# AlmondGod/diffusion-piano

Hardware: AMD Instinct MI355X
Metric: env steps/sec at 4096 parallel envs; qpos L∞ drift vs CPU MuJoCo (higher is better)
Workload: dtype f32; 1 GPU; 4096 envs/GPU crossing_field random-action rollout, 10 physics substeps per env-step, constraint forces by the primal Newton solve (friction loss, uncapped rows); envs_per_gpu=4096, song=crossing_field, parallelism=dp1

## Files before the change

### diffusion-piano_amd/csrc/collide_x.h

```cpp
#pragma once
#include "prims.h"

namespace ps {

struct XShape {
  int type;
  f3 c;
  float R[9];
  f3 p0, p1;
  float r;
  f3 hs;
  int v0, nv;
  f3 e0, e1;
  float er;
  const uint64_t* cells;
  const float4* cellv;
  float tie;
};

constexpr float SUP_TIE_HULL = 2e-6f;
constexpr float SUP_TIE_BOX = 1e-6f;
constexpr float SUP_TIE_CAP = 1e-6f;

__device__ __forceinline__ void x_shift(XShape& s, f3 o) {
  s.c = s.c - o;
  s.p0 = s.p0 - o;
  s.p1 = s.p1 - o;
  s.e0 = s.e0 - o;
  s.e1 = s.e1 - o;
}

__device__ __forceinline__ void quat_to_R(float w, float x, float y, float z, float* R) {
  const float n = rsqrtf(w * w + x * x + y * y + z * z);
  w *= n; x *= n; y *= n; z *= n;
  R[0] = 1.f - 2.f * (y * y + z * z); R[1] = 2.f * (x * y - w * z); R[2] = 2.f * (x * z + w * y);
  R[3] = 2.f * (x * y + w * z); R[4] = 1.f - 2.f * (x * x + z * z); R[5] = 2.f * (y * z - w * x);
  R[6] = 2.f * (x * z - w * y); R[7] = 2.f * (y * z + w * x); R[8] = 1.f - 2.f * (x * x + y * y);
}
__device__ __forceinline__ void R_to_quat(const float* R, float* q) {
  const float t = R[0] + R[4] + R[8];
  if (t > 0.f) {
    const float s = sqrtf(t + 1.f) * 2.f, i = 1.f / s;
    q[0] = 0.25f * s; q[1] = (R[7] - R[5]) * i; q[2] = (R[2] - R[6]) * i; q[3] = (R[3] - R[1]) * i;
  } else if (R[0] > R[4] && R[0] > R[8]) {
    const float s = sqrtf(1.f + R[0] - R[4] - R[8]) * 2.f, i = 1.f / s;
    q[0] = (R[7] - R[5]) * i; q[1] = 0.25f * s; q[2] = (R[1] + R[3]) * i; q[3] = (R[2] + R[6]) * i;
  } else if (R[4] > R[8]) {
    const float s = sqrtf(1.f + R[4] - R[0] - R[8]) * 2.f, i = 1.f / s;
    q[0] = (R[2] - R[6]) * i; q[1] = (R[1] + R[3]) * i; q[2] = 0.25f * s; q[3] = (R[5] + R[7]) * i;
  } else {
    const float s = sqrtf(1.f + R[8] - R[0] - R[4]) * 2.f, i = 1.f / s;
    q[0] = (R[3] - R[1]) * i; q[1] = (R[2] + R[6]) * i; q[2] = (R[5] + R[7]) * i; q[3] = 0.25f * s;
  }
}

__device__ __forceinline__ float sgn0f(float x) { return x > 0.f ? 1.f : (x < 0.f ? -1.f : 0.f); }
__device__ __forceinline__ f3 nrmz3(f3 a) {
  const float n = norm3(a);
  return n > 0.f ? a * (1.f / n) : a;
}

__device__ __forceinline__ int hull_cell(f3 d) {
  const float ex = fabsf(d.x), ey = fabsf(d.y), ez = fabsf(d.z);
  int ax;
  float mj, a, b;
  if (ex >= ey && ex >= ez) { ax = 0; mj = d.x; a = d.y; b = d.z; }
  else if (ey >= ez) { ax = 1; mj = d.y; a = d.z; b = d.x; }
  else { ax = 2; mj = d.z; a = d.x; b = d.y; }
  const float inv = 1.f / fabsf(mj), hg = 0.5f * XCG;
  const int ia = (int)fminf(fmaxf(fmaf(a, inv, 1.f) * hg, 0.f), XCG - 1.f);
  const int ib = (int)fminf(fmaxf(fmaf(b, inv, 1.f) * hg, 0.f), XCG - 1.f);
  return ((2 * ax + (mj < 0.f ? 1 : 0)) * XCG + ia) * XCG + ib;
}

__device__ __forceinline__ float sgn_tie(float x, float band) { return fabsf(x) <= band ? 0.f : sgn0f(x); }
__device__ __forceinline__ f3 x_support_local(const DevModel* __restrict__ m, const XShape& s, f3 d) {
  const f3 dl = mtv3(s.R, d);
  f3 loc;
  if (s.type == PS_GEOM_BOX) {
    const float band = SUP_TIE_BOX * fmaxf(fabsf(dl.x), fmaxf(fabsf(dl.y), fabsf(dl.z)));
    loc = mk3(sgn_tie(dl.x, band) * s.hs.x, sgn_tie(dl.y, band) * s.hs.y, sgn_tie(dl.z, band) * s.hs.z);
  } else if (s.cellv) {
    const bool zero = dl.x == 0.f && dl.y == 0.f && dl.z == 0.f;
    const float4* t = s.cellv + (zero ? XNCELL : hull_cell(dl)) * XCV;
    float4 v[XCV];
#pragma unroll
    for (int u = 0; u < XCV; u++) v[u] = t[u];
    const float tie = s.tie * norm3(dl);
    float bd = -INFINITY;
    loc = mk3(0.f, 0.f, 0.f);
#pragma unroll
    for (int u = 0; u < XCV; u++) {
      const float p = fmaf(dl.z, v[u].z, fmaf(dl.y, v[u].y, dl.x * v[u].x));
      if (p > bd + tie) { bd = p; loc = mk3(v[u].x, v[u].y, v[u].z); }
    }
  } else if (s.cells) {
    const bool zero = dl.x == 0.f && dl.y == 0.f && dl.z == 0.f;
    uint64_t msk = zero ? 1ull : s.cells[hull_cell(dl)];
    const float tie = s.tie * norm3(dl);
    float bd = -INFINITY;
    loc = mk3(0.f, 0.f, 0.f);
    while (msk) {
      bool ok[4];
      f3 v[4];
#pragma unroll
      for (int u = 0; u < 4; u++) {
        ok[u] = msk != 0ull;
        const int id = ok[u] ? __builtin_ctzll(msk) : 0;
        msk &= msk - 1ull;
        const float4 q = *reinterpret_cast<const float4*>(m->hull_v[s.v0 + id]);
        v[u] = mk3(q.x, q.y, q.z);
      }
#pragma unroll
      for (int u = 0; u < 4; u++) {
        const float p = fmaf(dl.z, v[u].z, fmaf(dl.y, v[u].y, dl.x * v[u].x));
        if (ok[u] && p > bd + tie) { bd = p; loc = v[u]; }
      }
    }
  } else {
    const float tie = s.tie * norm3(dl);
    float bd = -INFINITY;
    loc = mk3(0.f, 0.f, 0.f);
    for (int i0 = 0; i0 < s.nv; i0 += 8) {
      float4 v[8];
#pragma unroll
      for (int j = 0; j < 8; j++) v[j] = *reinterpret_cast<const float4*>(m->hull_v[s.v0 + min(i0 + j, s.nv - 1)]);
#pragma unroll
      for (int j = 0; j < 8; j++) {
        const float p = fmaf(dl.z, v[j].z, fmaf(dl.y, v[j].y, dl.x * v[j].x));
        if (i0 + j < s.nv && p > bd + tie) { bd = p; loc = mk3(v[j].x, v[j].y, v[j].z); }
      }
    }
  }
  return loc;
}
__device__ __forceinline__ f3 x_support(const DevModel* __restrict__ m, const XShape& s, f3 d) {
  if (s.type == 0) {
    const f3 ax = s.p1 - s.p0;
    const float dn = norm3(d);
    float da = dot3(ax, d);
    if (fabsf(da) <= SUP_TIE_CAP * norm3(ax) * dn) da = 0.f;
    const f3 base = da > 0.f ? s.p1 : (da < 0.f ? s.p0 : (s.p0 + s.p1) * 0.5f);
    return dn > 0.f ? base + d * (s.r / dn) : base;
  }
  return s.c + mv3(s.R, x_support_local(m, s, d));
}

constexpr float MPR_TOLF = 1e-6f;
constexpr int MPR_MAXITF = 50;
constexpr float MPR_EPSF = 2.220446049250313e-16f;
struct MprPt {
  f3 v, a, b;
};
__device__ __forceinline__ bool mpr_zero(float x) { return fabsf(x) < MPR_EPSF; }
__device__ __forceinline__ MprPt mpr_sup(const DevModel* __restrict__ m, const XShape& A, const XShape& B, f3 d) {
  MprPt p;
  p.a = x_support(m, A, d);
  p.b = x_support(m, B, d * -1.f);
  p.v = p.a - p.b;
  return p;
}
__device__ __forceinline__ float xchg1(float v) {
  return __int_as_float(__builtin_amdgcn_update_dpp(0, __float_as_int(v), 0xB1, 0xF, 0xF, false));
}
template <bool PAIR>
__device__ __forceinline__ MprPt mpr_sup_t(const DevModel* __restrict__ m, const XShape& A, const XShape& B,
                                           const XShape& O, bool role, f3 d) {
  if (!PAIR) return mpr_sup(m, A, B, d);
  const f3 mine = x_support(m, O, role ? d * -1.f : d);
  const f3 oth = mk3(xchg1(mine.x), xchg1(mine.y), xchg1(mine.z));
  MprPt p;
  p.a = role ? oth : mine;
  p.b = role ? mine : oth;
  p.v = p.a - p.b;
  return p;
}
__device__ __forceinline__ f3 portal_dir(const MprPt& p1, const MprPt& p2, const MprPt& p3) {
  return nrmz3(cross3(p2.v - p1.v, p3.v - p1.v));
}
__device__ __forceinline__ bool portal_reach_tol(const MprPt& p1, const MprPt& p2, const MprPt& p3, const MprPt& v4, f3 dir) {
  const float d4 = dot3(v4.v, dir);
  const float mn = fminf(d4 - dot3(p1.v, dir), fminf(d4 - dot3(p2.v, dir), d4 - dot3(p3.v, dir)));
  return mn <= MPR_TOLF;
}
__device__ __forceinline__ void expand_portal(const MprPt& p0, MprPt& p1, MprPt& p2, MprPt& p3, const MprPt& v4) {
  const f3 v4v0 = cross3(v4.v, p0.v);
  if (dot3(p1.v, v4v0) > 0.f) {
    if (dot3(p2.v, v4v0) > 0.f) p1 = v4; else p3 = v4;
  } else {
    if (dot3(p3.v, v4v0) > 0.f) p2 = v4; else p1 = v4;
  }
}
__device__ __forceinline__ f3 tri_closest_origin_d(f3 af, f3 bf, f3 cf) {
  const double ax = af.x, ay = af.y, az = af.z, bx = bf.x, by = bf.y, bz = bf.z, cx = cf.x, cy = cf.y, cz = cf.z;
  const double abx = bx - ax, aby = by - ay, abz = bz - az, acx = cx - ax, acy = cy - ay, acz = cz - az;
  const double d1 = -(abx * ax + aby * ay + abz * az), d2 = -(acx * ax + acy * ay + acz * az);
  if (d1 <= 0.0 && d2 <= 0.0) return af;
  const double d3 = -(abx * bx + aby * by + abz * bz), d4 = -(acx * bx + acy * by + acz * bz);
  if (d3 >= 0.0 && d4 <= d3) return bf;
  const double vc = d1 * d4 - d3 * d2;
  if (vc <= 0.0 && d1 >= 0.0 && d3 <= 0.0) {
    const double t = d1 / (d1 - d3);
    return mk3((float)(ax + abx * t), (float)(ay + aby * t), (float)(az + abz * t));
  }
  const double d5 = -(abx * cx + aby * cy + abz * cz), d6 = -(acx * cx + acy * cy + acz * cz);
  if (d6 >= 0.0 && d5 <= d6) return cf;
  const double vb = d5 * d2 - d1 * d6;
  if (vb <= 0.0 && d2 >= 0.0 && d6 <= 0.0) {
    const double t = d2 / (d2 - d6);
    return mk3((float)(ax + acx * t), (float)(ay + acy * t), (float)(az + acz * t));
  }
  const double va = d3 * d6 - d5 * d4;
  if (va <= 0.0 && (d4 - d3) >= 0.0 && (d5 - d6) >= 0.0) {
    const double t = (d4 - d3) / ((d4 - d3) + (d5 - d6));
    return mk3((float)(bx + (cx - bx) * t), (float)(by + (cy - by) * t), (float)(bz + (cz - bz) * t));
  }
  const double den = 1.0 / (va + vb + vc), v = vb * den, w = vc * den;
  return mk3((float)(ax + abx * v + acx * w), (float)(ay + aby * v + acy * w), (float)(az + abz * v + acz * w));
}
__device__ __forceinline__ f3 mpr_pos(const MprPt& p0, const MprPt& p1, const MprPt& p2, const MprPt& p3) {
  const f3 dir = portal_dir(p1, p2, p3);
  float b0 = dot3(cross3(p1.v, p2.v), p3.v), b1 = dot3(cross3(p3.v, p2.v), p0.v);
  float b2 = dot3(cross3(p0.v, p1.v), p3.v), b3 = dot3(cross3(p2.v, p1.v), p0.v);
  float sum = b0 + b1 + b2 + b3;
// ... 4 lines not shown
    b3 = dot3(cross3(p1.v, p2.v), dir);
    sum = b1 + b2 + b3;
  }
  const float inv = 1.f / sum;
  const f3 pa = p0.a * b0 + p1.a * b1 + p2.a * b2 + p3.a * b3;
  const f3 pb = p0.b * b0 + p1.b * b1 + p2.b * b2 + p3.b * b3;
  return (pa * inv + pb * inv) * 0.5f;
}
template <bool PAIR = false>
__device__ __forceinline__ int mpr_penetration(const DevModel* __restrict__ m, const XShape& A, const XShape& B,
                                               float* depth, f3* n, f3* pos, int* its = nullptr,
                                               const XShape* O = nullptr, bool role = false) {
  const XShape& own = PAIR ? *O : A;
  MprPt p0, p1, p2, p3;
  p0.a = A.c; p0.b = B.c; p0.v = A.c - B.c;
  if (p0.v.x == 0.f && p0.v.y == 0.f && p0.v.z == 0.f) p0.v.x += 10.f * MPR_EPSF;
  f3 dir = nrmz3(p0.v * -1.f);
  p1 = mpr_sup_t<PAIR>(m, A, B, own, role, dir);
  float dt = dot3(p1.v, dir);
  if (mpr_zero(dt) || dt < 0.f) return 0;
  dir = cross3(p0.v, p1.v);
  if (mpr_zero(dot3(dir, dir))) {
    *pos = (p1.a + p1.b) * 0.5f;
    if (p1.v.x == 0.f && p1.v.y == 0.f && p1.v.z == 0.f) { *depth = 0.f; *n = mk3(0.f, 0.f, 0.f); }
    else { *depth = norm3(p1.v); *n = nrmz3(p1.v); }
    return 1;
  }
  dir = nrmz3(dir);
  p2 = mpr_sup_t<PAIR>(m, A, B, own, role, dir);
  dt = dot3(p2.v, dir);
  if (mpr_zero(dt) || dt < 0.f) return 0;
  dir = nrmz3(cross3(p1.v - p0.v, p2.v - p0.v));
  if (dot3(dir, p0.v) > 0.f) { const MprPt t = p1; p1 = p2; p2 = t; dir = dir * -1.f; }
  for (int it = 0;; it++) {
    if (its) ++*its;
    if (it > 4 * MPR_MAXITF) return 0;
    p3 = mpr_sup_t<PAIR>(m, A, B, own, role, dir);
    dt = dot3(p3.v, dir);
    if (mpr_zero(dt) || dt < 0.f) return 0;
    bool cont = false;
    float t = dot3(cross3(p1.v, p3.v), p0.v);
    if (t < 0.f && !mpr_zero(t)) { p2 = p3; cont = true; }
    if (!cont) {
      t = dot3(cross3(p3.v, p2.v), p0.v);
      if (t < 0.f && !mpr_zero(t)) { p1 = p3; cont = true; }
    }
    if (!cont) break;
    dir = nrmz3(cross3(p1.v - p0.v, p2.v - p0.v));
  }
  for (int it = 0;; it++) {
    if (its) ++*its;
    if (it > 4 * MPR_MAXITF) return 0;
    dir = portal_dir(p1, p2, p3);
    dt = dot3(p1.v, dir);
    if (mpr_zero(dt) || dt > 0.f) break;
    const MprPt v4 = mpr_sup_t<PAIR>(m, A, B, own, role, dir);
    const float d4 = dot3(v4.v, dir);
    if (!(mpr_zero(d4) || d4 > 0.f) || portal_reach_tol(p1, p2, p3, v4, dir)) return 0;
    expand_portal(p0, p1, p2, p3, v4);
  }
  for (int it = 0;; it++) {
    if (its) ++*its;
    dir = portal_dir(p1, p2, p3);
    const MprPt v4 = mpr_sup_t<PAIR>(m, A, B, own, role, dir);
    if (portal_reach_tol(p1, p2, p3, v4, dir) || it > MPR_MAXITF) {
      const f3 cp = tri_closest_origin_d(p1.v, p2.v, p3.v);
      *depth = norm3(cp);
      *n = mpr_zero(*depth) ? dir : cp * (1.f / *depth);
      *pos = mpr_pos(p0, p1, p2, p3);
      return 1;
    }
    expand_portal(p0, p1, p2, p3, v4);
  }
}

struct d3 {
  double x, y, z;
};
__device__ __forceinline__ d3 mkd3(double a, double b, double c) { return {a, b, c}; }
__device__ __forceinline__ d3 tod3(f3 a) { return {a.x, a.y, a.z}; }
__device__ __forceinline__ f3 tof3(d3 a) { return mk3((float)a.x, (float)a.y, (float)a.z); }
__device__ __forceinline__ d3 operator+(d3 a, d3 b) { return {a.x + b.x, a.y + b.y, a.z + b.z}; }
__device__ __forceinline__ d3 operator-(d3 a, d3 b) { return {a.x - b.x, a.y - b.y, a.z - b.z}; }
__device__ __forceinline__ d3 operator*(d3 a, double s) { return {a.x * s, a.y * s, a.z * s}; }
__device__ __forceinline__ double dotd(d3 a, d3 b) { return a.x * b.x + a.y * b.y + a.z * b.z; }
__device__ __forceinline__ d3 crossd(d3 a, d3 b) {
  return {a.y * b.z - a.z * b.y, a.z * b.x - a.x * b.z, a.x * b.y - a.y * b.x};
}
#ifndef PS_MPR_FASTN
#define PS_MPR_FASTN 1
#endif
__device__ __forceinline__ double rsqrtd(double x) {
  const double r = (double)__frsqrt_rn((float)x);
  return r * (1.5 - 0.5 * x * r * r);
}
__device__ __forceinline__ d3 nrmzd(d3 a) {
  const double n2 = dotd(a, a);
  if (PS_MPR_FASTN && n2 > 1e-30 && n2 < 1e30) return a * rsqrtd(n2);
  const double n = sqrt(n2);
  return n > 0.0 ? a * (1.0 / n) : a;
}
__device__ __forceinline__ bool mpr_zerod(double x) { return fabs(x) < 2.220446049250313e-16; }
__device__ __forceinline__ d3 x_support_d(const DevModel* __restrict__ m, const XShape& s, d3 d) {
  if (s.type == 0) {
    const d3 p0 = tod3(s.p0), p1 = tod3(s.p1), ax = p1 - p0;
    const double dd = dotd(d, d);
// ... 16 lines not shown
struct MprPtD {
  d3 v, a, b;
};
__device__ __forceinline__ double xchg1d(double v) {
  const long long u = __double_as_longlong(v);
  const int lo = __builtin_amdgcn_update_dpp(0, (int)(u & 0xffffffffll), 0xB1, 0xF, 0xF, false);
  const int hi = __builtin_amdgcn_update_dpp(0, (int)(u >> 32), 0xB1, 0xF, 0xF, false);
  return __longlong_as_double(((long long)hi << 32) | (unsigned int)lo);
}
template <bool PAIR>
__device__ __forceinline__ MprPtD mpr_sup_d(const DevModel* __restrict__ m, const XShape& A, const XShape& B,
                                            const XShape& O, bool role, d3 d) {
  MprPtD p;
  if (!PAIR) {
    p.a = x_support_d(m, A, d);
    p.b = x_support_d(m, B, d * -1.0);
  } else {
    const d3 mine = x_support_d(m, O, role ? d * -1.0 : d);
    const d3 oth = mkd3(xchg1d(mine.x), xchg1d(mine.y), xchg1d(mine.z));
    p.a = role ? oth : mine;
    p.b = role ? mine : oth;
  }
  p.v = p.a - p.b;
  return p;
}
__device__ __forceinline__ d3 portal_dir_d(const MprPtD& p1, const MprPtD& p2, const MprPtD& p3) {
  return nrmzd(crossd(p2.v - p1.v, p3.v - p1.v));
}
__device__ __forceinline__ bool portal_reach_tol_d(const MprPtD& p1, const MprPtD& p2, const MprPtD& p3,
                                                   const MprPtD& v4, d3 dir) {
  const double d4 = dotd(v4.v, dir);
  return fmin(d4 - dotd(p1.v, dir), fmin(d4 - dotd(p2.v, dir), d4 - dotd(p3.v, dir))) <= 1e-6;
}
__device__ __forceinline__ void expand_portal_d(const MprPtD& p0, MprPtD& p1, MprPtD& p2, MprPtD& p3, const MprPtD& v4) {
  const d3 v4v0 = crossd(v4.v, p0.v);
  if (dotd(p1.v, v4v0) > 0.0) {
    if (dotd(p2.v, v4v0) > 0.0) p1 = v4; else p3 = v4;
  } else {
    if (dotd(p3.v, v4v0) > 0.0) p2 = v4; else p1 = v4;
  }
}
__device__ __forceinline__ d3 tri_closest_origin_dd(d3 a, d3 b, d3 c) {
  const d3 ab = b - a, ac = c - a;
  const double d1 = -dotd(ab, a), d2 = -dotd(ac, a);
  if (d1 <= 0.0 && d2 <= 0.0) return a;
  const double d3_ = -dotd(ab, b), d4 = -dotd(ac, b);
  if (d3_ >= 0.0 && d4 <= d3_) return b;
  const double vc = d1 * d4 - d3_ * d2;
  if (vc <= 0.0 && d1 >= 0.0 && d3_ <= 0.0) return a + ab * (d1 / (d1 - d3_));
  const double d5 = -dotd(ab, c), d6 = -dotd(ac, c);
  if (d6 >= 0.0 && d5 <= d6) return c;
  const double vb = d5 * d2 - d1 * d6;
  if (vb <= 0.0 && d2 >= 0.0 && d6 <= 0.0) return a + ac * (d2 / (d2 - d6));
  const double va = d3_ * d6 - d5 * d4;
  if (va <= 0.0 && (d4 - d3_) >= 0.0 && (d5 - d6) >= 0.0) return b + (c - b) * ((d4 - d3_) / ((d4 - d3_) + (d5 - d6)));
  const double den = 1.0 / (va + vb + vc);
  return a + ab * (vb * den) + ac * (vc * den);
}
__device__ __forceinline__ d3 mpr_pos_d(const MprPtD& p0, const MprPtD& p1, const MprPtD& p2, const MprPtD& p3) {
  const d3 dir = portal_dir_d(p1, p2, p3);
  double b0 = dotd(crossd(p1.v, p2.v), p3.v), b1 = dotd(crossd(p3.v, p2.v), p0.v);
  double b2 = dotd(crossd(p0.v, p1.v), p3.v), b3 = dotd(crossd(p2.v, p1.v), p0.v);
  double sum = b0 + b1 + b2 + b3;
  if (mpr_zerod(sum) || sum < 0.0) {
    b0 = 0.0;
    b1 = dotd(crossd(p2.v, p3.v), dir);
    b2 = dotd(crossd(p3.v, p1.v), dir);
    b3 = dotd(crossd(p1.v, p2.v), dir);
    sum = b1 + b2 + b3;
  }
  const double inv = 1.0 / sum;
  const d3 pa = p0.a * b0 + p1.a * b1 + p2.a * b2 + p3.a * b3;
  const d3 pb = p0.b * b0 + p1.b * b1 + p2.b * b2 + p3.b * b3;
  return (pa * inv + pb * inv) * 0.5;
}
template <bool PAIR = false>
__device__ __forceinline__ int mpr_penetration_d(const DevModel* __restrict__ m, const XShape& A, const XShape& B,
                                                 float* depth, f3* n, f3* pos, int* its = nullptr,
                                                 const XShape* O = nullptr, bool role = false) {
  const XShape& own = PAIR ? *O : A;
  MprPtD p0, p1, p2, p3;
  p0.a = tod3(A.c); p0.b = tod3(B.c); p0.v = p0.a - p0.b;
  if (p0.v.x == 0.0 && p0.v.y == 0.0 && p0.v.z == 0.0) p0.v.x += 10.0 * 2.220446049250313e-16;
  d3 dir = nrmzd(p0.v * -1.0);
  p1 = mpr_sup_d<PAIR>(m, A, B, own, role, dir);
  double dt = dotd(p1.v, dir);
  if (mpr_zerod(dt) || dt < 0.0) return 0;
  dir = crossd(p0.v, p1.v);
  if (mpr_zerod(dotd(dir, dir))) {
    *pos = tof3((p1.a + p1.b) * 0.5);
    if (p1.v.x == 0.0 && p1.v.y == 0.0 && p1.v.z == 0.0) { *depth = 0.f; *n = mk3(0.f, 0.f, 0.f); }
    else { *depth = (float)sqrt(dotd(p1.v, p1.v)); *n = tof3(nrmzd(p1.v)); }
    return 1;
  }
  dir = nrmzd(dir);
  p2 = mpr_sup_d<PAIR>(m, A, B, own, role, dir);
  dt = dotd(p2.v, dir);
  if (mpr_zerod(dt) || dt < 0.0) return 0;
  dir = nrmzd(crossd(p1.v - p0.v, p2.v - p0.v));
  if (dotd(dir, p0.v) > 0.0) { const MprPtD t = p1; p1 = p2; p2 = t; dir = dir * -1.0; }
  for (int it = 0;; it++) {
    if (its) ++*its;
    if (it > 4 * MPR_MAXITF) return 0;
    p3 = mpr_sup_d<PAIR>(m, A, B, own, role, dir);
    dt = dotd(p3.v, dir);
    if (mpr_zerod(dt) || dt < 0.0) return 0;
    bool cont = false;
    double t = dotd(crossd(p1.v, p3.v), p0.v);
    if (t < 0.0 && !mpr_zerod(t)) { p2 = p3; cont = true; }
    if (!cont) {
      t = dotd(crossd(p3.v, p2.v), p0.v);
      if (t < 0.0 && !mpr_zerod(t)) { p1 = p3; cont = true; }
    }
    if (!cont) break;
    dir = nrmzd(crossd(p1.v - p0.v, p2.v - p0.v));
  }
  for (int it = 0;; it++) {
    if (its) ++*its;
    if (it > 4 * MPR_MAXITF) return 0;
    dir = portal_dir_d(p1, p2, p3);
    dt = dotd(p1.v, dir);
    if (mpr_zerod(dt) || dt > 0.0) break;
    const MprPtD v4 = mpr_sup_d<PAIR>(m, A, B, own, role, dir);
    const double d4 = dotd(v4.v, dir);
    if (!(mpr_zerod(d4) || d4 > 0.0) || portal_reach_tol_d(p1, p2, p3, v4, dir)) return 0;
    expand_portal_d(p0, p1, p2, p3, v4);
  }
  for (int it = 0;; it++) {
    if (its) ++*its;
    dir = portal_dir_d(p1, p2, p3);
    const MprPtD v4 = mpr_sup_d<PAIR>(m, A, B, own, role, dir);
    if (portal_reach_tol_d(p1, p2, p3, v4, dir) || it > MPR_MAXITF) {
      const d3 cp = tri_closest_origin_dd(p1.v, p2.v, p3.v);
      const double dep = sqrt(dotd(cp, cp));
      *depth = (float)dep;
      *n = tof3(mpr_zerod(dep) ? dir : cp * (1.0 / dep));
      *pos = tof3(mpr_pos_d(p0, p1, p2, p3));
      return 1;
    }
    expand_portal_d(p0, p1, p2, p3, v4);
  }
}

template <int N>
__device__ __forceinline__ void put3(f3 (&a)[N], int i, f3 v) {
#pragma unroll
  for (int j = 0; j < N; j++)
    if (j == i) a[j] = v;
}
template <int N>
__device__ __forceinline__ f3 get3(const f3 (&a)[N], int i) {
  f3 r = a[0];
#pragma unroll
  for (int j = 1; j < N; j++)
    if (j == i) r = a[j];
  return r;
}
__device__ __forceinline__ f3 rcol(const float* R, int i) { return mk3(R[i], R[3 + i], R[6 + i]); }
__device__ __forceinline__ float f3c(f3 a, int i) { return i == 0 ? a.x : (i == 1 ? a.y : a.z); }

constexpr int BB_MAXPT = 4;
__device__ __forceinline__ int box_box(const XShape& A, const XShape& B, f3 (&pos)[BB_MAXPT], float (&dist)[BB_MAXPT],
                                       f3* nout) {
  f3 a[3], b[3];
#pragma unroll
  for (int i = 0; i < 3; i++) { a[i] = rcol(A.R, i); b[i] = rcol(B.R, i); }
  const f3 t = B.c - A.c;
  float best = INFINITY;
  int bax = -1;
  f3 bn = mk3(0.f, 0.f, 0.f);
#pragma unroll
  for (int k = 0; k < 15; k++) {
    f3 L;
    if (k < 3) L = a[k];
// ... 245 lines not shown
```

### diffusion-piano_amd/csrc/kernel_v2.inc

```

#ifdef PS_TIMING
#define NPHASE 56
enum : int { TS_FINAL = 52, TS_FINAL_SKIP = 53 };
#define TARG , uint64_t *tacc, uint64_t &tlast
#define TPASS , tacc, tlast
#define TSTAMP(slot)                                     \
  do {                                                   \
    __syncthreads();                                     \
    uint64_t t_ = __builtin_amdgcn_s_memtime();         \
    tacc[slot] += t_ - tlast;                            \
    tlast = t_;                                          \
  } while (0)
__device__ uint64_t* g_timing = nullptr;
#else
#define TSTAMP(slot) \
  do {               \
  } while (0)
#define TARG
#define TPASS
#endif

#ifdef PS_CHECK_A
__device__ int g_dbg_count = 0;
#endif
enum : int { BX_R = 0, BX_CP = 0, BX_O = 10, BX_W = 13, BX_AL = 16, BX_AC = 19, BX_F = 22, BX_N = 25, BXS = 28 };
static_assert(NKB == 64, "collide2 stages one key-range bucket per lane");
constexpr int FROW = 2 * MAXDEP + 2;
__device__ __forceinline__ int tri(int r, int s) { return s * (s + 1) / 2 + r; }

constexpr int NSL = 28;
struct NewtonLDS {
  union {
    struct {
      float Jc[3 * MAXCON][YS];
      float P[68];
      float Bd[3][64];
// ... 177 lines not shown
                                                 int cap) {
  const int e = c - NGT;
  const f3 ctr = ld3(S.xg[e]);
  const float rb = m->x_rb[e];
  const float lo[3] = {ctr.x - rb, ctr.y - rb, ctr.z - rb}, hi[3] = {ctr.x + rb, ctr.y + rb, ctr.z + rb};
  int n = 0;
  if (!(lo[2] > m->key_top_zmax || hi[0] < m->piano_xmin || lo[0] > m->piano_xmax)) {
    const int b0 = min(max((int)floorf((lo[1] - 1e-5f - m->kb_y0) * m->kb_inv), 0), NKB - 1);
    const int b1 = min(max((int)floorf((hi[1] + 1e-5f - m->kb_y0) * m->kb_inv), 0), NKB - 1);
    const int k0 = S.kb[0][b0], k1 = S.kb[1][b1];
    for (int k = k0; k < k1; k++) {
      const float* g = S.kg[k];
      if (lo[2] > g[13] || hi[0] < g[9] || lo[0] > g[10] || hi[1] < g[11] || lo[1] > g[12]) continue;
      {
        const float cq = S.kc[k], sq = S.ks[k];
        const f3 al = ld3(g + 6), hs = ld3(g + 3);
        const f3 d = ctr - (ld3(g) + al);
        const f3 l = mk3(cq * d.x - sq * d.z + al.x, d.y + al.y, sq * d.x + cq * d.z + al.z);
        const f3 e = mk3(fmaxf(fabsf(l.x) - hs.x, 0.f), fmaxf(fabsf(l.y) - hs.y, 0.f), fmaxf(fabsf(l.z) - hs.z, 0.f));
        if (dot3(e, e) > rb * rb) continue;
      }
      if (emit && n < cap) emit[n] = (uint16_t)((c << 8) | k);
      n++;
    }
  }
  const f3 bc = ld3(m->base_pos), bh = ld3(m->base_half);
  if (hi[0] < bc.x - bh.x || lo[0] > bc.x + bh.x || hi[1] < bc.y - bh.y || lo[1] > bc.y + bh.y ||
      hi[2] < bc.z - bh.z || lo[2] > bc.z + bh.z)
    return n;
  if (emit && n < cap) emit[n] = (uint16_t)((c << 8) | BASEKEY);
  return n + 1;
}

__device__ __forceinline__ XShape coll_shape(const DevModel* __restrict__ m, const Shared& S, int g) {
  XShape s;
  s.cells = nullptr;
  s.cellv = nullptr;
  s.v0 = s.nv = 0;
  s.r = 0.f;
  s.er = 0.f;
  s.tie = 0.f;
  s.hs = mk3(0.f, 0.f, 0.f);
  if (g < NGT) {
    s.type = 0;
    s.p0 = ld3(&S.cap[g][0]);
    s.p1 = ld3(&S.cap[g][3]);
    s.r = S.cap[g][6];
    s.c = (s.p0 + s.p1) * 0.5f;
    s.e0 = s.e1 = s.c;
#pragma unroll
    for (int i = 0; i < 9; i++) s.R[i] = (i % 4 == 0) ? 1.f : 0.f;
  } else {
    const int e = g - NGT;
    s.type = m->x_type[e];
    s.c = ld3(S.xg[e]);
#pragma unroll
    for (int i = 0; i < 9; i++) s.R[i] = S.xg[e][3 + i];
    s.hs = ld3(m->x_hs[e]);
    s.v0 = m->x_v0[e];
    s.nv = m->x_nv[e];
    s.p0 = s.p1 = s.e0 = s.e1 = s.c;
    if (s.type == PS_GEOM_HULL) {
      s.cells = m->x_cell[e];
      s.cellv = m->x_cellv_ok[e] ? reinterpret_cast<const float4*>(&m->x_cellv[e][0][0][0]) : nullptr;
      s.e0 = s.c + mv3(s.R, ld3(&m->x_ec[e][0]));
      s.e1 = s.c + mv3(s.R, ld3(&m->x_ec[e][3]));
      s.er = m->x_ec[e][6];
      s.tie = SUP_TIE_HULL * m->x_rb[e];
    }
  }
  return s;
}

__device__ __forceinline__ void x_pair_shapes(const DevModel* __restrict__ m, const Shared& S, int ga, int gb, int key,
                                              XShape& A, XShape& B, int& kind, int& ckey) {
  B = coll_shape(m, S, gb);
  kind = 2;
  ckey = -1;
  if (ga < 0) {
    A.type = PS_GEOM_BOX;
    A.cells = nullptr;
    A.cellv = nullptr;
    A.v0 = A.nv = 0;
    A.r = 0.f;
    if (key == BASEKEY) {
      kind = 1;
      A.c = ld3(m->base_pos);
      A.hs = ld3(m->base_half);
#pragma unroll
      for (int i = 0; i < 9; i++) A.R[i] = (i % 4 == 0) ? 1.f : 0.f;
    } else {
      kind = 0;
      ckey = key;
      const float* g = S.kg[key];
      const float cq = S.kc[key], sq = S.ks[key];
      const float R[9] = {cq, 0.f, sq, 0.f, 1.f, 0.f, -sq, 0.f, cq};
#pragma unroll
      for (int i = 0; i < 9; i++) A.R[i] = R[i];
      const f3 al = ld3(g + 6), an = ld3(g) + al;
      A.c = an + mv3(R, al * -1.f);
      A.hs = ld3(g + 3);
    }
    A.p0 = A.p1 = A.e0 = A.e1 = A.c;
    A.er = 0.f;
    A.tie = 0.f;
  } else {
    A = coll_shape(m, S, ga);
  }
}

constexpr int XHH = 0x8000;
static_assert(NGT + 2 * NX <= 128, "pair list entry fields");
__device__ __forceinline__ void x_entry(int pk, int& ga, int& gb, int& key) {
  const bool hh = pk & XHH;
  ga = hh ? pk & 255 : -1;
  key = hh ? -1 : pk & 255;
  gb = (pk >> 8) & 127;
}
#ifndef PS_XREFINE_ATTR
#define PS_XREFINE_ATTR __noinline__
#endif
#ifndef PS_XPAIRS_ATTR
#define PS_XPAIRS_ATTR __noinline__
#endif
template <int WPE>
__device__ PS_XREFINE_ATTR int x_refine(const DevModel* __restrict__ m, const Shared* Sp, uint16_t* list, int n,
                                     int lane) {
  const Shared& S = *Sp;
  int kept = 0;
  for (int r0 = 0; r0 < n; r0 += 64) {
    const int i = r0 + lane;
    const int pk = i < n ? (int)list[i] : 0;
    bool keep = false;
    if (i < n) {
      XShape A, B;
      int kind, ckey, ga, gb, key;
      x_entry(pk, ga, gb, key);
      x_pair_shapes(m, S, ga, gb, key, A, B, kind, ckey);
      keep = !x_apart(A, B);
    }
    const uint64_t mask = __ballot(keep);
    wsync();
    if (keep) list[kept + lanes_below(mask, lane)] = (uint16_t)pk;
    kept += __popcll(mask);
    wsync();
  }
  return kept;
}

template <int WPE>
__device__ PS_XPAIRS_ATTR int x_pairs(const DevModel* __restrict__ m, const Shared* Sp, bool act, int ga, int gb, int key,
                                    Contact* out, int base, int maxc, int lane,
                                    int* its = nullptr) {
  const Shared& S = *Sp;
  if (!act) { ga = -1; gb = NGT; key = BASEKEY; }
  XShape A, B;
  int kind, ckey;
  x_pair_shapes(m, S, ga, gb, key, A, B, kind, ckey);
  int g1 = ga < 0 ? -1 : ga, g2 = gb;
  f3 pos[BB_MAXPT], nrm[BB_MAXPT];
  float dist[BB_MAXPT];
  bool swap = false;
  int nit = 0;
  const bool role = lane & 1;
  int cnt = act ? x_narrow_local<true>(m, A, B, pos, dist, nrm, swap, its ? &nit : nullptr, role) : 0;
  if (its) {
    its[0] = -(int)wave_min(-(float)nit);
    its[1] = __popcll(__ballot(act && !role));
    its[2] = __popcll(__ballot(act && !role && cnt > 0));
    its[3] = wave_sum_i(act && !role ? nit : 0);
    its[4] = wave_sum_i(act && !role && cnt > 0 ? nit : 0);
  }
  if (role) cnt = 0;
  if (swap) {
    g1 = gb;
    g2 = ga;
  }
  int rt;
  const int slot = base + small_excl_scan<3>(cnt, lane, &rt);
  {
#pragma unroll
    for (int j = 0; j < BB_MAXPT; j++) {
      if (j < cnt && slot + j < maxc) {
        Contact& cc = out[slot + j];
        st3(cc.pos, pos[j]);
        st3(cc.n, nrm[j]);
        cc.dist = dist[j];
        f3 t1, t2;
        make_frame(nrm[j], &t1, &t2);
        st3(cc.t1, t1);
        st3(cc.t2, t2);
        cc.kind = kind;
        cc.key = ckey;
        cc.g1 = g1;
        cc.g2 = g2;
      }
    }
  }
  return rt;
}

constexpr int NSTAGE = 32, STAGE_OFF = 2 * 256;
static_assert(STAGE_OFF >= 2 * NSTAGE, "candidate list overlaps the staging area");
constexpr int CPL = 8, CSTAGE_OFF = 2 * NGT * CPL;
// ... 172 lines not shown
          const int p = p0 + 64 * u + lane;
          const int pk = pks[u];
          const int ga = pk & 255, gb = pk >> 8;
          const float rba = __shfl(x_rbl, ga, 64), rbb = __shfl(x_rbl, gb, 64);
          bool pass = false;
          if (p < nxp) {
            f3 c2[2];
            float rad = 0.f;
#pragma unroll
            for (int q = 0; q < 2; q++) {
              const int g = q ? gb : ga;
              if (g < NGT) {
                c2[q] = (ld3(&S.cap[g][0]) + ld3(&S.cap[g][3])) * 0.5f;
                rad += S.cap[g][6] + S.cap[g][7];
              } else {
                c2[q] = ld3(S.xg[g - NGT]);
                rad += q ? rbb : rba;
              }
            }
            pass = norm3(c2[0] - c2[1]) <= rad;
          }
          const uint64_t mask = __ballot(pass);
          const int at = nl + lanes_below(mask, lane);
          if (pass && at < MAXCAND) cand[at] = (uint16_t)(pk | XHH);
          nl = min(nl + __popcll(mask), MAXCAND);
        }
      }
#ifdef PS_TIMING
      tacc[45] += nl;
#endif
    }
    wsync();
    TSTAMP(35);
    nl = x_refine<WPE>(m, &S, cand, nl, lane);
#ifdef PS_TIMING
    tacc[42] += nl > 0;
#endif
    TSTAMP(36);
    for (int q0 = 0; q0 < nl && base < maxc; q0 += 32) {
      const int q = q0 + (lane >> 1);
      int ga, gb, key;
      x_entry(q < nl ? (int)cand[q] : 0, ga, gb, key);
#ifdef PS_TIMING
      int its[5] = {0, 0, 0, 0, 0};
      base += x_pairs<WPE>(m, &S, q < nl, ga, gb, key, S.con, base, maxc, lane, its);
      tacc[30] += its[0];
      tacc[31] += 1;
      tacc[38] += its[1];
      tacc[39] += its[2];
      tacc[40] += its[3];
      tacc[41] += its[4];
#else
      base += x_pairs<WPE>(m, &S, q < nl, ga, gb, key, S.con, base, maxc, lane);
#endif
    }
    TSTAMP(37);
  }
  if (lane == 0) S.ncon = base < maxc ? base : maxc;
  wsync();
  return base;
}

template <bool XG>
__device__ __forceinline__ bool fore_near(const DevModel* __restrict__ m, const Shared& S, int lane) {
  const int nf = m->nfore;
  if (nf < 0) return true;
  bool pass = false;
  if (lane < nf) {
    const int pk = m->fore_pair[lane];
    const int ga = pk & 255, gb = pk >> 8;
    if (ga < NGT && gb < NGT) {
      const float *A = S.cap[ga], *B = S.cap[gb];
      const float reach = A[6] + B[6] + 1e-4f;
      float d2 = 0.f;
#pragma unroll
      for (int i = 0; i < 3; i++) {
        const float alo = fminf(A[i], A[3 + i]), ahi = fmaxf(A[i], A[3 + i]);
        const float blo = fminf(B[i], B[3 + i]), bhi = fmaxf(B[i], B[3 + i]);
        const float gap = fmaxf(0.f, fmaxf(alo - bhi, blo - ahi));
        d2 += gap * gap;
      }
      pass = !(d2 > reach * reach);
    } else if (XG) {
      f3 c2[2];
      float rad = 0.f;
#pragma unroll
// ... 1304 lines not shown
```

### diffusion-piano_amd/csrc/prims.h

```cpp
#pragma once
#include <hip/hip_runtime.h>
#include <math.h>
#include <stdint.h>

#include "devmodel.h"

namespace ps {

#define MINIMP 0.0001f
#define MAXIMP 0.9999f
#define MINVALF 1e-15f
#define KEY_THRESHOLD 0.00872665f
#define SUSTAIN_THRESHOLD 0.5f

struct f3 {
  float x, y, z;
};
__device__ __forceinline__ f3 mk3(float a, float b, float c) { return {a, b, c}; }
__device__ __forceinline__ f3 ld3(const float* p) { return {p[0], p[1], p[2]}; }
__device__ __forceinline__ void st3(float* p, f3 a) { p[0] = a.x; p[1] = a.y; p[2] = a.z; }
__device__ __forceinline__ f3 operator+(f3 a, f3 b) { return {a.x + b.x, a.y + b.y, a.z + b.z}; }
__device__ __forceinline__ f3 operator-(f3 a, f3 b) { return {a.x - b.x, a.y - b.y, a.z - b.z}; }
__device__ __forceinline__ f3 operator*(f3 a, float s) { return {a.x * s, a.y * s, a.z * s}; }
__device__ __forceinline__ float dot3(f3 a, f3 b) { return a.x * b.x + a.y * b.y + a.z * b.z; }
__device__ __forceinline__ f3 cross3(f3 a, f3 b) {
  return {a.y * b.z - a.z * b.y, a.z * b.x - a.x * b.z, a.x * b.y - a.y * b.x};
}
__device__ __forceinline__ float norm3(f3 a) { return sqrtf(dot3(a, a)); }
__device__ __forceinline__ float clampf(float x, float lo, float hi) { return x < lo ? lo : (x > hi ? hi : x); }
__device__ __forceinline__ f3 mv3(const float* R, f3 a) {
  return {R[0] * a.x + R[1] * a.y + R[2] * a.z, R[3] * a.x + R[4] * a.y + R[5] * a.z,
          R[6] * a.x + R[7] * a.y + R[8] * a.z};
}
__device__ __forceinline__ f3 mtv3(const float* R, f3 a) {
  return {R[0] * a.x + R[3] * a.y + R[6] * a.z, R[1] * a.x + R[4] * a.y + R[7] * a.z,
          R[2] * a.x + R[5] * a.y + R[8] * a.z};
}
__device__ __forceinline__ void mm3(const float* A, const float* B, float* C) {
#pragma unroll
  for (int i = 0; i < 3; i++)
#pragma unroll
    for (int j = 0; j < 3; j++) C[3 * i + j] = A[3 * i] * B[j] + A[3 * i + 1] * B[3 + j] + A[3 * i + 2] * B[6 + j];
}
__device__ __forceinline__ f3 sym_mv(const float* I, f3 a) {
  return {I[0] * a.x + I[3] * a.y + I[4] * a.z, I[3] * a.x + I[1] * a.y + I[5] * a.z,
          I[4] * a.x + I[5] * a.y + I[2] * a.z};
}

__device__ __forceinline__ float wave_sum(float v) {
  int x = __float_as_int(v);
  v += __int_as_float(__builtin_amdgcn_update_dpp(0, x, 0x111, 0xF, 0xF, false));
  x = __float_as_int(v);
  v += __int_as_float(__builtin_amdgcn_update_dpp(0, x, 0x112, 0xF, 0xF, false));
// ... 351 lines not shown
```

Baseline: 966,100 env-steps/s.

## Use explicit address spaces in narrowphase and fuse MPR phases into one loop

Pointers to the model and to the shared scratch used by the hull-collision path now carry explicit global and LDS address-space qualifiers. This lets the compiler emit direct global/LDS loads instead of flat loads inside the noinline x_refine/x_pairs functions. The three sequential MPR loops (discovery, portal refinement, penetration) are merged into one phase-driven loop with index-based portal replacement, so the support call sits at a single site and divergent lanes in different phases can share it. It also adds timing counters for mixed-type waves and no-hit waves. The phase-merged loop adds some branching and bookkeeping per iteration and could change iteration-count behaviour at the edges.

```diff
diff --git a/diffusion-piano_amd/csrc/collide_x.h b/diffusion-piano_amd/csrc/collide_x.h
--- a/diffusion-piano_amd/csrc/collide_x.h
+++ b/diffusion-piano_amd/csrc/collide_x.h
@@ -13,8 +13,8 @@
   int v0, nv;
   f3 e0, e1;
   float er;
-  const uint64_t* cells;
-  const float4* cellv;
+  const PS_GLB uint64_t* cells;
+  const PS_GLB f4g* cellv;
   float tie;
 };
 
@@ -75,6 +75,7 @@
 
 __device__ __forceinline__ float sgn_tie(float x, float band) { return fabsf(x) <= band ? 0.f : sgn0f(x); }
 __device__ __forceinline__ f3 x_support_local(const DevModel* __restrict__ m, const XShape& s, f3 d) {
+  const PS_GLB float(*hull_v)[4] = ((const PS_GLB DevModel*)m)->hull_v;
   const f3 dl = mtv3(s.R, d);
   f3 loc;
   if (s.type == PS_GEOM_BOX) {
@@ -82,8 +83,8 @@
     loc = mk3(sgn_tie(dl.x, band) * s.hs.x, sgn_tie(dl.y, band) * s.hs.y, sgn_tie(dl.z, band) * s.hs.z);
   } else if (s.cellv) {
     const bool zero = dl.x == 0.f && dl.y == 0.f && dl.z == 0.f;
-    const float4* t = s.cellv + (zero ? XNCELL : hull_cell(dl)) * XCV;
-    float4 v[XCV];
+    const PS_GLB f4g* t = s.cellv + (zero ? XNCELL : hull_cell(dl)) * XCV;
+    f4g v[XCV];
 #pragma unroll
     for (int u = 0; u < XCV; u++) v[u] = t[u];
     const float tie = s.tie * norm3(dl);
@@ -108,7 +109,7 @@
         ok[u] = msk != 0ull;
         const int id = ok[u] ? __builtin_ctzll(msk) : 0;
         msk &= msk - 1ull;
-        const float4 q = *reinterpret_cast<const float4*>(m->hull_v[s.v0 + id]);
+        const f4g q = *reinterpret_cast<const PS_GLB f4g*>(hull_v[s.v0 + id]);
         v[u] = mk3(q.x, q.y, q.z);
       }
 #pragma unroll
@@ -122,9 +123,9 @@
     float bd = -INFINITY;
     loc = mk3(0.f, 0.f, 0.f);
     for (int i0 = 0; i0 < s.nv; i0 += 8) {
-      float4 v[8];
-#pragma unroll
-      for (int j = 0; j < 8; j++) v[j] = *reinterpret_cast<const float4*>(m->hull_v[s.v0 + min(i0 + j, s.nv - 1)]);
+      f4g v[8];
+#pragma unroll
+      for (int j = 0; j < 8; j++) v[j] = *reinterpret_cast<const PS_GLB f4g*>(hull_v[s.v0 + min(i0 + j, s.nv - 1)]);
 #pragma unroll
       for (int j = 0; j < 8; j++) {
         const float p = fmaf(dl.z, v[j].z, fmaf(dl.y, v[j].y, dl.x * v[j].x));
@@ -183,13 +184,11 @@
   const float mn = fminf(d4 - dot3(p1.v, dir), fminf(d4 - dot3(p2.v, dir), d4 - dot3(p3.v, dir)));
   return mn <= MPR_TOLF;
 }
-__device__ __forceinline__ void expand_portal(const MprPt& p0, MprPt& p1, MprPt& p2, MprPt& p3, const MprPt& v4) {
+__device__ __forceinline__ int expand_portal_idx(const MprPt& p0, const MprPt& p1, const MprPt& p2, const MprPt& p3,
+                                                 const MprPt& v4) {
   const f3 v4v0 = cross3(v4.v, p0.v);
-  if (dot3(p1.v, v4v0) > 0.f) {
-    if (dot3(p2.v, v4v0) > 0.f) p1 = v4; else p3 = v4;
-  } else {
-    if (dot3(p3.v, v4v0) > 0.f) p2 = v4; else p1 = v4;
-  }
+  if (dot3(p1.v, v4v0) > 0.f) return dot3(p2.v, v4v0) > 0.f ? 1 : 3;
+  return dot3(p3.v, v4v0) > 0.f ? 2 : 1;
 }
 __device__ __forceinline__ f3 tri_closest_origin_d(f3 af, f3 bf, f3 cf) {
   const double ax = af.x, ay = af.y, az = af.z, bx = bf.x, by = bf.y, bz = bf.z, cx = cf.x, cy = cf.y, cz = cf.z;
@@ -260,46 +259,56 @@
   if (mpr_zero(dt) || dt < 0.f) return 0;
   dir = nrmz3(cross3(p1.v - p0.v, p2.v - p0.v));
   if (dot3(dir, p0.v) > 0.f) { const MprPt t = p1; p1 = p2; p2 = t; dir = dir * -1.f; }
+  int phase = 0;
   for (int it = 0;; it++) {
     if (its) ++*its;
-    if (it > 4 * MPR_MAXITF) return 0;
-    p3 = mpr_sup_t<PAIR>(m, A, B, own, role, dir);
-    dt = dot3(p3.v, dir);
-    if (mpr_zero(dt) || dt < 0.f) return 0;
-    bool cont = false;
-    float t = dot3(cross3(p1.v, p3.v), p0.v);
-    if (t < 0.f && !mpr_zero(t)) { p2 = p3; cont = true; }
-    if (!cont) {
-      t = dot3(cross3(p3.v, p2.v), p0.v);
-      if (t < 0.f && !mpr_zero(t)) { p1 = p3; cont = true; }
-    }
-    if (!cont) break;
-    dir = nrmz3(cross3(p1.v - p0.v, p2.v - p0.v));
-  }
-  for (int it = 0;; it++) {
-    if (its) ++*its;
-    if (it > 4 * MPR_MAXITF) return 0;
-    dir = portal_dir(p1, p2, p3);
-    dt = dot3(p1.v, dir);
-    if (mpr_zero(dt) || dt > 0.f) break;
+    if (phase != 2 && it > 4 * MPR_MAXITF) return 0;
+    if (phase != 0) {
+      dir = portal_dir(p1, p2, p3);
+      if (phase == 1) {
+        dt = dot3(p1.v, dir);
+        if (mpr_zero(dt) || dt > 0.f) {
+          phase = 2;
+          it = 0;
+          if (its) ++*its;
+        }
+      }
+    }
     const MprPt v4 = mpr_sup_t<PAIR>(m, A, B, own, role, dir);
-    const float d4 = dot3(v4.v, dir);
-    if (!(mpr_zero(d4) || d4 > 0.f) || portal_reach_tol(p1, p2, p3, v4, dir)) return 0;
-    expand_portal(p0, p1, p2, p3, v4);
-  }
-  for (int it = 0;; it++) {
-    if (its) ++*its;
-    dir = portal_dir(p1, p2, p3);
-    const MprPt v4 = mpr_sup_t<PAIR>(m, A, B, own, role, dir);
-    if (portal_reach_tol(p1, p2, p3, v4, dir) || it > MPR_MAXITF) {
-      const f3 cp = tri_closest_origin_d(p1.v, p2.v, p3.v);
-      *depth = norm3(cp);
-      *n = mpr_zero(*depth) ? dir : cp * (1.f / *depth);
-      *pos = mpr_pos(p0, p1, p2, p3);
-      return 1;
-    }
-    expand_portal(p0, p1, p2, p3, v4);
-  }
+    const bool disc = phase == 0;
+    int rp = 3;
+    if (disc) {
+      dt = dot3(v4.v, dir);
+      if (mpr_zero(dt) || dt < 0.f) return 0;
+      float t = dot3(cross3(p1.v, v4.v), p0.v);
+      if (t < 0.f && !mpr_zero(t)) rp = 2;
+      else {
+        t = dot3(cross3(v4.v, p2.v), p0.v);
+        if (t < 0.f && !mpr_zero(t)) rp = 1;
+      }
+    } else {
+      const bool reach = portal_reach_tol(p1, p2, p3, v4, dir);
+      if (phase == 1) {
+        const float d4 = dot3(v4.v, dir);
+        if (!(mpr_zero(d4) || d4 > 0.f) || reach) return 0;
+      } else if (reach || it > MPR_MAXITF) {
+        break;
+      }
+      rp = expand_portal_idx(p0, p1, p2, p3, v4);
+    }
+    if (rp == 1) p1 = v4;
+    if (rp == 2) p2 = v4;
+    if (rp == 3 || disc) p3 = v4;
+    if (disc) {
+      if (rp == 3) { phase = 1; it = -1; }
+      else dir = nrmz3(cross3(p1.v - p0.v, p2.v - p0.v));
+    }
+  }
+  const f3 cp = tri_closest_origin_d(p1.v, p2.v, p3.v);
+  *depth = norm3(cp);
+  *n = mpr_zero(*depth) ? dir : cp * (1.f / *depth);
+  *pos = mpr_pos(p0, p1, p2, p3);
+  return 1;
 }
 
 struct d3 {
@@ -382,13 +391,11 @@
   const double d4 = dotd(v4.v, dir);
   return fmin(d4 - dotd(p1.v, dir), fmin(d4 - dotd(p2.v, dir), d4 - dotd(p3.v, dir))) <= 1e-6;
 }
-__device__ __forceinline__ void expand_portal_d(const MprPtD& p0, MprPtD& p1, MprPtD& p2, MprPtD& p3, const MprPtD& v4) {
+__device__ __forceinline__ int expand_portal_idx_d(const MprPtD& p0, const MprPtD& p1, const MprPtD& p2, const MprPtD& p3,
+                                                   const MprPtD& v4) {
   const d3 v4v0 = crossd(v4.v, p0.v);
-  if (dotd(p1.v, v4v0) > 0.0) {
-    if (dotd(p2.v, v4v0) > 0.0) p1 = v4; else p3 = v4;
-  } else {
-    if (dotd(p3.v, v4v0) > 0.0) p2 = v4; else p1 = v4;
-  }
+  if (dotd(p1.v, v4v0) > 0.0) return dotd(p2.v, v4v0) > 0.0 ? 1 : 3;
+  return dotd(p3.v, v4v0) > 0.0 ? 2 : 1;
 }
 __device__ __forceinline__ d3 tri_closest_origin_dd(d3 a, d3 b, d3 c) {
   const d3 ab = b - a, ac = c - a;
@@ -449,47 +456,57 @@
   if (mpr_zerod(dt) || dt < 0.0) return 0;
   dir = nrmzd(crossd(p1.v - p0.v, p2.v - p0.v));
   if (dotd(dir, p0.v) > 0.0) { const MprPtD t = p1; p1 = p2; p2 = t; dir = dir * -1.0; }
+  int phase = 0;
   for (int it = 0;; it++) {
     if (its) ++*its;
-    if (it > 4 * MPR_MAXITF) return 0;
-    p3 = mpr_sup_d<PAIR>(m, A, B, own, role, dir);
-    dt = dotd(p3.v, dir);
-    if (mpr_zerod(dt) || dt < 0.0) return 0;
-    bool cont = false;
-    double t = dotd(crossd(p1.v, p3.v), p0.v);
-    if (t < 0.0 && !mpr_zerod(t)) { p2 = p3; cont = true; }
-    if (!cont) {
-      t = dotd(crossd(p3.v, p2.v), p0.v);
-      if (t < 0.0 && !mpr_zerod(t)) { p1 = p3; cont = true; }
-    }
-    if (!cont) break;
-    dir = nrmzd(crossd(p1.v - p0.v, p2.v - p0.v));
-  }
-  for (int it = 0;; it++) {
-    if (its) ++*its;
-    if (it > 4 * MPR_MAXITF) return 0;
-    dir = portal_dir_d(p1, p2, p3);
-    dt = dotd(p1.v, dir);
-    if (mpr_zerod(dt) || dt > 0.0) break;
+    if (phase != 2 && it > 4 * MPR_MAXITF) return 0;
+    if (phase != 0) {
+      dir = portal_dir_d(p1, p2, p3);
+      if (phase == 1) {
+        dt = dotd(p1.v, dir);
+        if (mpr_zerod(dt) || dt > 0.0) {
+          phase = 2;
+          it = 0;
+          if (its) ++*its;
+        }
+      }
+    }
     const MprPtD v4 = mpr_sup_d<PAIR>(m, A, B, own, role, dir);
-    const double d4 = dotd(v4.v, dir);
-    if (!(mpr_zerod(d4) || d4 > 0.0) || portal_reach_tol_d(p1, p2, p3, v4, dir)) return 0;
-    expand_portal_d(p0, p1, p2, p3, v4);
-  }
-  for (int it = 0;; it++) {
-    if (its) ++*its;
-    dir = portal_dir_d(p1, p2, p3);
-    const MprPtD v4 = mpr_sup_d<PAIR>(m, A, B, own, role, dir);
-    if (portal_reach_tol_d(p1, p2, p3, v4, dir) || it > MPR_MAXITF) {
-      const d3 cp = tri_closest_origin_dd(p1.v, p2.v, p3.v);
-      const double dep = sqrt(dotd(cp, cp));
-      *depth = (float)dep;
-      *n = tof3(mpr_zerod(dep) ? dir : cp * (1.0 / dep));
-      *pos = tof3(mpr_pos_d(p0, p1, p2, p3));
-      return 1;
-    }
-    expand_portal_d(p0, p1, p2, p3, v4);
-  }
+    const bool disc = phase == 0;
+    int rp = 3;
+    if (disc) {
+      dt = dotd(v4.v, dir);
+      if (mpr_zerod(dt) || dt < 0.0) return 0;
+      double t = dotd(crossd(p1.v, v4.v), p0.v);
+      if (t < 0.0 && !mpr_zerod(t)) rp = 2;
+      else {
+        t = dotd(crossd(v4.v, p2.v), p0.v);
+        if (t < 0.0 && !mpr_zerod(t)) rp = 1;
+      }
+    } else {
+      const bool reach = portal_reach_tol_d(p1, p2, p3, v4, dir);
+      if (phase == 1) {
+        const double d4 = dotd(v4.v, dir);
+        if (!(mpr_zerod(d4) || d4 > 0.0) || reach) return 0;
+      } else if (reach || it > MPR_MAXITF) {
+        break;
+      }
+      rp = expand_portal_idx_d(p0, p1, p2, p3, v4);
+    }
+    if (rp == 1) p1 = v4;
+    if (rp == 2) p2 = v4;
+    if (rp == 3 || disc) p3 = v4;
+    if (disc) {
+      if (rp == 3) { phase = 1; it = -1; }
+      else dir = nrmzd(crossd(p1.v - p0.v, p2.v - p0.v));
+    }
+  }
+  const d3 cp = tri_closest_origin_dd(p1.v, p2.v, p3.v);
+  const double dep = sqrt(dotd(cp, cp));
+  *depth = (float)dep;
+  *n = tof3(mpr_zerod(dep) ? dir : cp * (1.0 / dep));
+  *pos = tof3(mpr_pos_d(p0, p1, p2, p3));
+  return 1;
 }
 
 template <int N>
diff --git a/diffusion-piano_amd/csrc/kernel_v2.inc b/diffusion-piano_amd/csrc/kernel_v2.inc
--- a/diffusion-piano_amd/csrc/kernel_v2.inc
+++ b/diffusion-piano_amd/csrc/kernel_v2.inc
@@ -2,6 +2,7 @@
 #ifdef PS_TIMING
 #define NPHASE 56
 enum : int { TS_FINAL = 52, TS_FINAL_SKIP = 53 };
+enum : int { TS_XMIXED = 54, TS_XNOHIT = 55 };
 #define TARG , uint64_t *tacc, uint64_t &tlast
 #define TPASS , tacc, tlast
 #define TSTAMP(slot)                                     \
@@ -245,7 +246,7 @@
   return n + 1;
 }
 
-__device__ __forceinline__ XShape coll_shape(const DevModel* __restrict__ m, const Shared& S, int g) {
+__device__ __forceinline__ XShape coll_shape(const PS_GLB DevModel* m, const PS_LDS Shared* S, int g) {
   XShape s;
   s.cells = nullptr;
   s.cellv = nullptr;
@@ -256,9 +257,9 @@
   s.hs = mk3(0.f, 0.f, 0.f);
   if (g < NGT) {
     s.type = 0;
-    s.p0 = ld3(&S.cap[g][0]);
-    s.p1 = ld3(&S.cap[g][3]);
-    s.r = S.cap[g][6];
+    s.p0 = ld3(&S->cap[g][0]);
+    s.p1 = ld3(&S->cap[g][3]);
+    s.r = S->cap[g][6];
     s.c = (s.p0 + s.p1) * 0.5f;
     s.e0 = s.e1 = s.c;
 #pragma unroll
@@ -266,16 +267,16 @@
   } else {
     const int e = g - NGT;
     s.type = m->x_type[e];
-    s.c = ld3(S.xg[e]);
-#pragma unroll
-    for (int i = 0; i < 9; i++) s.R[i] = S.xg[e][3 + i];
+    s.c = ld3(S->xg[e]);
+#pragma unroll
+    for (int i = 0; i < 9; i++) s.R[i] = S->xg[e][3 + i];
     s.hs = ld3(m->x_hs[e]);
     s.v0 = m->x_v0[e];
     s.nv = m->x_nv[e];
     s.p0 = s.p1 = s.e0 = s.e1 = s.c;
     if (s.type == PS_GEOM_HULL) {
       s.cells = m->x_cell[e];
-      s.cellv = m->x_cellv_ok[e] ? reinterpret_cast<const float4*>(&m->x_cellv[e][0][0][0]) : nullptr;
+      s.cellv = m->x_cellv_ok[e] ? reinterpret_cast<const PS_GLB f4g*>(&m->x_cellv[e][0][0][0]) : nullptr;
       s.e0 = s.c + mv3(s.R, ld3(&m->x_ec[e][0]));
       s.e1 = s.c + mv3(s.R, ld3(&m->x_ec[e][3]));
       s.er = m->x_ec[e][6];
@@ -285,7 +286,7 @@
   return s;
 }
 
-__device__ __forceinline__ void x_pair_shapes(const DevModel* __restrict__ m, const Shared& S, int ga, int gb, int key,
+__device__ __forceinline__ void x_pair_shapes(const PS_GLB DevModel* m, const PS_LDS Shared* S, int ga, int gb, int key,
                                               XShape& A, XShape& B, int& kind, int& ckey) {
   B = coll_shape(m, S, gb);
   kind = 2;
@@ -305,8 +306,8 @@
     } else {
       kind = 0;
       ckey = key;
-      const float* g = S.kg[key];
-      const float cq = S.kc[key], sq = S.ks[key];
+      const PS_LDS float* g = S->kg[key];
+      const float cq = S->kc[key], sq = S->ks[key];
       const float R[9] = {cq, 0.f, sq, 0.f, 1.f, 0.f, -sq, 0.f, cq};
 #pragma unroll
       for (int i = 0; i < 9; i++) A.R[i] = R[i];
@@ -337,24 +338,23 @@
 #define PS_XPAIRS_ATTR __noinline__
 #endif
 template <int WPE>
-__device__ PS_XREFINE_ATTR int x_refine(const DevModel* __restrict__ m, const Shared* Sp, uint16_t* list, int n,
+__device__ PS_XREFINE_ATTR int x_refine(const PS_GLB DevModel* mg, const PS_LDS Shared* S, PS_LDS uint16_t* ll, int n,
                                      int lane) {
-  const Shared& S = *Sp;
   int kept = 0;
   for (int r0 = 0; r0 < n; r0 += 64) {
     const int i = r0 + lane;
-    const int pk = i < n ? (int)list[i] : 0;
+    const int pk = i < n ? (int)ll[i] : 0;
     bool keep = false;
     if (i < n) {
       XShape A, B;
       int kind, ckey, ga, gb, key;
       x_entry(pk, ga, gb, key);
-      x_pair_shapes(m, S, ga, gb, key, A, B, kind, ckey);
+      x_pair_shapes(mg, S, ga, gb, key, A, B, kind, ckey);
       keep = !x_apart(A, B);
     }
     const uint64_t mask = __ballot(keep);
     wsync();
-    if (keep) list[kept + lanes_below(mask, lane)] = (uint16_t)pk;
+    if (keep) ll[kept + lanes_below(mask, lane)] = (uint16_t)pk;
     kept += __popcll(mask);
     wsync();
   }
@@ -362,14 +362,14 @@
 }
 
 template <int WPE>
-__device__ PS_XPAIRS_ATTR int x_pairs(const DevModel* __restrict__ m, const Shared* Sp, bool act, int ga, int gb, int key,
+__device__ PS_XPAIRS_ATTR int x_pairs(const PS_GLB DevModel* mg, const PS_LDS Shared* S, bool act, int ga, int gb, int key,
                                     Contact* out, int base, int maxc, int lane,
                                     int* its = nullptr) {
-  const Shared& S = *Sp;
   if (!act) { ga = -1; gb = NGT; key = BASEKEY; }
   XShape A, B;
   int kind, ckey;
-  x_pair_shapes(m, S, ga, gb, key, A, B, kind, ckey);
+  x_pair_shapes(mg, S, ga, gb, key, A, B, kind, ckey);
+  const DevModel* m = (const DevModel*)mg;
   int g1 = ga < 0 ? -1 : ga, g2 = gb;
   f3 pos[BB_MAXPT], nrm[BB_MAXPT];
   float dist[BB_MAXPT];
@@ -383,6 +383,11 @@
     its[2] = __popcll(__ballot(act && !role && cnt > 0));
     its[3] = wave_sum_i(act && !role ? nit : 0);
     its[4] = wave_sum_i(act && !role && cnt > 0 ? nit : 0);
+#ifdef PS_TIMING
+    const bool mpr = !((A.type == 0 || A.type == PS_GEOM_BOX) && B.type == PS_GEOM_BOX);
+    its[5] = __ballot(act && mpr) != 0ull && __ballot(act && !mpr) != 0ull;
+    its[6] = __ballot(act && !role && cnt > 0) == 0ull;
+#endif
   }
   if (role) cnt = 0;
   if (swap) {
@@ -621,7 +626,9 @@
     }
     wsync();
     TSTAMP(35);
-    nl = x_refine<WPE>(m, &S, cand, nl, lane);
+    const PS_GLB DevModel* mg = (const PS_GLB DevModel*)m;
+    const PS_LDS Shared* Sl = (const PS_LDS Shared*)&S;
+    nl = x_refine<WPE>(mg, Sl, (PS_LDS uint16_t*)cand, nl, lane);
 #ifdef PS_TIMING
     tacc[42] += nl > 0;
 #endif
@@ -631,16 +638,18 @@
       int ga, gb, key;
       x_entry(q < nl ? (int)cand[q] : 0, ga, gb, key);
 #ifdef PS_TIMING
-      int its[5] = {0, 0, 0, 0, 0};
-      base += x_pairs<WPE>(m, &S, q < nl, ga, gb, key, S.con, base, maxc, lane, its);
+      int its[7] = {0, 0, 0, 0, 0, 0, 0};
+      base += x_pairs<WPE>(mg, Sl, q < nl, ga, gb, key, S.con, base, maxc, lane, its);
       tacc[30] += its[0];
       tacc[31] += 1;
       tacc[38] += its[1];
       tacc[39] += its[2];
       tacc[40] += its[3];
       tacc[41] += its[4];
+      tacc[TS_XMIXED] += its[5];
+      tacc[TS_XNOHIT] += its[6];
 #else
-      base += x_pairs<WPE>(m, &S, q < nl, ga, gb, key, S.con, base, maxc, lane);
+      base += x_pairs<WPE>(mg, Sl, q < nl, ga, gb, key, S.con, base, maxc, lane);
 #endif
     }
     TSTAMP(37);
diff --git a/diffusion-piano_amd/csrc/prims.h b/diffusion-piano_amd/csrc/prims.h
--- a/diffusion-piano_amd/csrc/prims.h
+++ b/diffusion-piano_amd/csrc/prims.h
@@ -19,6 +19,11 @@
 __device__ __forceinline__ f3 mk3(float a, float b, float c) { return {a, b, c}; }
 __device__ __forceinline__ f3 ld3(const float* p) { return {p[0], p[1], p[2]}; }
 __device__ __forceinline__ void st3(float* p, f3 a) { p[0] = a.x; p[1] = a.y; p[2] = a.z; }
+#define PS_LDS __attribute__((address_space(3)))
+#define PS_GLB __attribute__((address_space(1)))
+__device__ __forceinline__ f3 ld3(const PS_LDS float* p) { return {p[0], p[1], p[2]}; }
+__device__ __forceinline__ f3 ld3(const PS_GLB float* p) { return {p[0], p[1], p[2]}; }
+typedef float f4g __attribute__((ext_vector_type(4)));
 __device__ __forceinline__ f3 operator+(f3 a, f3 b) { return {a.x + b.x, a.y + b.y, a.z + b.z}; }
 __device__ __forceinline__ f3 operator-(f3 a, f3 b) { return {a.x - b.x, a.y - b.y, a.z - b.z}; }
 __device__ __forceinline__ f3 operator*(f3 a, float s) { return {a.x * s, a.y * s, a.z * s}; }
```

Measured after the change: 987,700 env-steps/s, median of 6. +2.2%, better.
